# databricks/spark-sklearn

Measured on NVIDIA H100. Metric: candidate-fits/sec, higher is better.
Workload: dtype f64

## Files before the change

### include/b200gs.h

```cpp
#ifndef B200GS_H
#define B200GS_H

#include <stdint.h>

#ifdef __cplusplus
extern "C" {
#endif

typedef struct gs_handle gs_handle;

enum gs_status {
    GS_OK = 0,
    GS_ERR_CUDA = -1,
    GS_ERR_ARG = -2,
    GS_ERR_NO_DATA = -3,
    GS_ERR_UNSUPPORTED = -4,
    GS_ERR_NUMERIC = -5
};

enum gs_kernel { GS_KERNEL_LINEAR = 0, GS_KERNEL_RBF = 1 };
enum gs_dtype { GS_F32 = 0, GS_F64 = 1 };

enum gs_flags {
    GS_RETURN_TRAIN = 1,
// ... 52 lines not shown
                    double *coef_out, int32_t *n_iter);

int gs_set_targets_f64(gs_handle *h, const double *y);
int gs_svr(gs_handle *h, int32_t n_cand, const int32_t *kernel, const double *C, const double *epsilon, const double *gamma,
           double tol, int32_t max_iter, uint32_t flags, double *test_scores, double *train_scores, int32_t *n_iter,
           int32_t *n_sv, float *fit_ms, float *score_ms);
int gs_svr_refit(gs_handle *h, int32_t kernel, double C, double epsilon, double gamma, double tol, int32_t max_iter,
                 uint32_t flags, double *coef, double *rho, int32_t *n_iter);

int gs_debug_gram(gs_handle *h, double *S_out, double *xsq_out);
int gs_debug_kernel_matrix(gs_handle *h, int32_t kernel, double gamma, float *K_out);

int gs_debug_gemm_nt(gs_handle *h, const float *A, int32_t M, const float *B, int32_t N, int32_t K, float *C);

double gs_svc_predicted_iterations(int32_t kernel, double C, double gamma, int32_t d);
int32_t gs_svc_cluster_count(const double *cost_desc, int32_t n, int32_t sm_count);
void gs_svc_schedule(const double *cost_desc, int32_t n, int32_t sm_count, int32_t *n_cluster, int32_t *n_exclusive);
double gs_svc_simulate(const double *cost_desc, int32_t n, int32_t sm_count, int32_t n_cluster, int32_t n_exclusive);

typedef struct gs_profile {
    float ms_total;
    float ms_h2d;
    float ms_gram;
    float ms_kernel_matrix;
    float ms_solve;
    float ms_score;
    int64_t launches;
    int64_t smo_iterations;
    double solve_bytes;
    double gram_flops;
// ... 13 lines not shown
```

### spark_sklearn_b200/csrc/api.cu

```cuda
#include "common.cuh"
#include <algorithm>
#include <cmath>
#include <cstring>
#include <cstdio>
#include <cstdlib>
#include <map>
#include <mutex>
#include <queue>
#include <numeric>

static std::string g_create_error;

double gs_score_from_counts(int kind, int pos_class, int n_classes, const int *cnt)
{
    auto sup = [&](int c) { return (double)cnt[c * 3 + 0]; };
    auto tp = [&](int c) { return (double)cnt[c * 3 + 1]; };
    auto prd = [&](int c) { return (double)cnt[c * 3 + 2]; };
    auto f1c = [&](int c) { const double den = sup(c) + prd(c); return den > 0 ? 2.0 * tp(c) / den : 0.0; };
    double n = 0, correct = 0;
    for (int c = 0; c < n_classes; c++) { n += sup(c); correct += tp(c); }
    if (!(n > 0)) return NAN;
    switch (kind) {
    case GS_SCORE_DEFAULT: return correct / n;
    case GS_SCORE_BALANCED_ACCURACY: {
// ... 258 lines not shown
    GS_CUDA(cudaMemcpyAsync(h->dTe.p, h->te_mask.data(), (size_t)n * 16, cudaMemcpyHostToDevice, h->stream));
    GS_CUDA(cudaMemcpyAsync(h->dTr.p, h->tr_mask.data(), (size_t)n * 16, cudaMemcpyHostToDevice, h->stream));
    GS_CUDA(cudaStreamSynchronize(h->stream));
    h->prof.h2d_bytes += n * 32;
    return GS_OK;
}

extern "C" double gs_svc_predicted_iterations(int32_t kernel, double C, double gamma, int32_t d)
{
    if (kernel != GS_KERNEL_RBF) return C;
    const double gd = gamma * (double)d;
    if (!(gd > 0)) return C;
    return std::min(4.0 + 10.3 * std::pow(C * gd, 0.95), 9.0 + 7.3 / gd);
}

extern "C" int32_t gs_svc_cluster_count(const double *cost_desc, int32_t n, int32_t sm_count)
{
    if (!cost_desc || n < 2 || sm_count < 4) return 0;
    double total = 0;
    for (int q = 0; q < n; q++) total += cost_desc[q];
    const int nmax = std::min(n - 1, sm_count / 4);
    double best = 0, clustered = 0;
    int pick = 0;
    for (int k = 0; k <= nmax; k++) {
        const double f = std::max({(total + clustered) / sm_count, 0.9 * cost_desc[k], k > 0 ? 0.5 * cost_desc[0] : 0.0});
        if (k == 0 || f < 0.97 * best) { best = f; pick = k; }
        clustered += cost_desc[k];
    }
    return pick;
}
// ... 235 lines not shown
    if (!refit && h->score_kind != GS_SCORE_DEFAULT) {
        const int kd = h->score_kind;
        if (kd == GS_SCORE_NEG_MSE || kd == GS_SCORE_NEG_RMSE) { gs_set_error(h, "gs_svc: regression scorer on a classifier"); return GS_ERR_ARG; }
        if ((kd == GS_SCORE_ROC_AUC || kd == GS_SCORE_F1 || kd == GS_SCORE_PRECISION || kd == GS_SCORE_RECALL) && nc != 2) {
            gs_set_error(h, "gs_svc: this scorer is defined for binary problems only"); return GS_ERR_UNSUPPORTED;
        }
        if (h->score_pos >= nc) { gs_set_error(h, "gs_svc: positive class out of range"); return GS_ERR_ARG; }
    }
    int64_t total_iter = 0;
    double solve_bytes = 0;

    for (int g0 = 0; g0 < n_groups; g0 += gpb) {
        const int g1 = std::min(n_groups, g0 + gpb);
        if (const int rc = search.kernel_matrices(g0, g1)) return rc;
        std::vector<SmoProblem> probs;
        std::vector<int> prob_task, group_first(g1 - g0 + 1, 0);
        std::vector<VoteTask> vtasks;
        std::vector<int> vtask_id;
        for (int g = g0; g < g1; g++) {
            group_first[g - g0] = (int)probs.size();
            for (int t : search.group_tasks[g]) {
                const int c = t / n_splits, k = t % n_splits;
                vtasks.push_back(VoteTask{(int)probs.size(), refit ? -100 : k});
                vtask_id.push_back(t);
                for (int p = 0; p < n_pairs; p++) {
                    const size_t s = (size_t)k * n_pairs + p;
                    SmoProblem P;
                    memset(&P, 0, sizeof P);
                    P.K = h->dK.as<float>() + (size_t)(g - g0) * n * ldk;
                    P.qd = search.groups[g].first == GS_KERNEL_LINEAR ? h->dXsq.as<double>() : nullptr;
                    P.rows = d_rows + sp_off[s];
// ... 2 lines not shown
                    for (int e = 0; e < 4; e++) { P.seg_start[e] = sp_seg[s * 8 + e]; P.seg_len[e] = sp_seg[s * 8 + 4 + e]; }
                    P.n_pos = sp_npos[s];
                    P.ldk = ldk; P.C = Cv[c]; P.Cn = Cv[c]; P.eps = tol; P.max_iter = max_iter;
                    if (h->class_w_sets > 0) {
                        const double *cw = &h->class_w[(size_t)(h->class_w_sets == 1 ? 0 : k) * nc];
                        int a_ = 0, b_ = 0, q_ = 0;
                        for (int a = 0; a < nc; a++) for (int b = a + 1; b < nc; b++, q_++) if (q_ == p) { a_ = a; b_ = b; }
                        P.C = Cv[c] * cw[a_]; P.Cn = Cv[c] * cw[b_];
                    }
                    P.shrinking = (flags & GS_NO_SHRINKING) ? 0 : 1;
                    P.guard = search.d_guard;
                    P.nslots = 0;
                    for (int e = 0; e < P.nseg; e++) P.nslots += P.seg_len[e];
                    probs.push_back(P);
                    prob_task.push_back(t);
                }
            }
        }
        group_first[g1 - g0] = (int)probs.size();
        const int np = (int)probs.size();
        if (const int rc = search.workspaces(probs)) return rc;
        GS_CUDA(h->dWork[6].reserve((size_t)np * sizeof(SmoProblem) + (size_t)np * 4 + vtasks.size() * (sizeof(VoteTask) + 16) + 256));
        std::vector<double> cost(np);
        for (int q = 0; q < np; q++) {
            const int t = prob_task[q];
            const auto &grp = search.groups[search.task_group[t]];
            cost[q] = gs_svc_predicted_iterations(grp.first, Cv[t / n_splits], grp.second, (int32_t)d) * (double)probs[q].l;
        }
        std::vector<int> order(np);
        std::iota(order.begin(), order.end(), 0);
        std::stable_sort(order.begin(), order.end(), [&](int a, int b) { return cost[a] > cost[b]; });
        unsigned char *dmeta = h->dWork[6].as<unsigned char>();
        SmoProblem *d_probs = (SmoProblem *)dmeta;
        int *d_order = (int *)(dmeta + (size_t)np * sizeof(SmoProblem));
        size_t off = (size_t)np * sizeof(SmoProblem) + (size_t)np * 4;
        off = (off + 15) & ~(size_t)15;
        VoteTask *d_vt = (VoteTask *)(dmeta + off);
        off += vtasks.size() * sizeof(VoteTask);
        off = (off + 15) & ~(size_t)15;
        int *d_counts = (int *)(dmeta + off);
        GS_CUDA(cudaMemcpyAsync(d_probs, probs.data(), (size_t)np * sizeof(SmoProblem), cudaMemcpyHostToDevice, st));
        GS_CUDA(cudaMemcpyAsync(d_order, order.data(), (size_t)np * 4, cudaMemcpyHostToDevice, st));
        GS_CUDA(cudaMemcpyAsync(d_vt, vtasks.data(), vtasks.size() * sizeof(VoteTask), cudaMemcpyHostToDevice, st));
        GS_CUDA(cudaMemsetAsync(d_counts, 0, vtasks.size() * 16, st));
        GS_CUDA(cudaMemsetAsync(h->dWork[3].p, 0, (size_t)np * n * 8, st));
        pf.h2d_bytes += (size_t)np * sizeof(SmoProblem) + (size_t)np * 4 + vtasks.size() * sizeof(VoteTask);
        search.tm.mark(4);
        std::string why;
        int max_slots = 0;
        bool lean_ok = lmax < 16383 && !(getenv("B200GS_SMO_LEAN") && atoi(getenv("B200GS_SMO_LEAN")) == 0);
        for (int q = 0; q < np && lean_ok; q++) {
            lean_ok = probs[q].nseg > 0 && probs[q].nslots <= smo_lean_max_slots();
            max_slots = std::max(max_slots, probs[q].nslots);
        }
        auto launch_single = [&](const int *ord, int cnt, cudaStream_t s_, bool exclusive) -> cudaError_t {
            for (int inst = search.fast ? 1 : 0; inst >= 0; inst--) {
                const cudaError_t e = lean_ok ? launch_smo_lean(d_probs, ord, cnt, max_slots, inst == 1, exclusive, s_)
                                              : launch_smo(d_probs, ord, cnt, lmax, inst == 1, (int)ldk, s_, &why);
                if (e != cudaSuccess) return e;
                pf.launches++;
            }
            return cudaSuccess;
        };
        int cl = 0, n_cl = 0, n_ex = 0;
        if (lmax > 2048) {
            if (np * 8 <= h->sm_count) { cl = 8; n_cl = np; }
            else if (np * 4 <= h->sm_count) { cl = 4; n_cl = np; }
            else if (np * 2 <= h->sm_count) { cl = 2; n_cl = np; }
            else {
                std::vector<double> sorted_cost(np);
                for (int q = 0; q < np; q++) sorted_cost[q] = cost[order[q]];
                if (lean_ok) gs_svc_schedule(sorted_cost.data(), np, h->sm_count, &n_cl, &n_ex);
                else n_cl = gs_svc_cluster_count(sorted_cost.data(), np, h->sm_count);
                if (n_cl > 0) cl = 4;
            }
        }
        if (const char *e = getenv("B200GS_SMO_CLUSTER")) { cl = atoi(e); if (n_cl == 0) n_cl = std::max(1, np * 6 / 100); }
        if (const char *e = getenv("B200GS_SMO_CLUSTER_N")) n_cl = std::min(np, atoi(e));
        if (!(cl == 2 || cl == 4 || cl == 8) || lmax > smo_colown_max_rows(cl) || lmax <= 2048) n_cl = 0;
        if (const char *e = getenv("B200GS_SMO_EXCLUSIVE_N")) n_ex = atoi(e);
        if (!lean_ok) n_ex = 0;
        n_ex = std::max(0, std::min(n_ex, np - n_cl));
        if (n_cl > 0 || n_ex > 0) {
            cudaEvent_t ready = h->evp.get();
            cudaEventRecord(ready, st);
            cudaError_t ce = cudaSuccess;
            if (n_cl > 0) {
                for (int inst = search.fast ? 1 : 0; inst >= 0 && ce == cudaSuccess; inst--) {
                    ce = launch_smo_colown(d_probs, d_order, n_cl, lmax, cl, inst == 1, st);
                    pf.launches++;
                }
                if (ce != cudaSuccess) { gs_set_error(h, std::string("launch_smo_colown: ") + cudaGetErrorString(ce)); return GS_ERR_CUDA; }
            }
            if (n_ex > 0) {
                cudaEvent_t done = h->evp.get();
                cudaStreamWaitEvent(h->stream_hi, ready, 0);
                launch_delay(30000, h->stream_hi);
// ... 39 lines not shown
                GS_CUDA(cudaMemcpyAsync(score_raw.data(), d_auc, (size_t)nvt * 32, cudaMemcpyDeviceToHost, st));
            } else {
                GS_CUDA(h->dScore.reserve((size_t)nvt * 2 * nc * 3 * 4));
                GS_CUDA(cudaMemsetAsync(h->dScore.p, 0, (size_t)nvt * 2 * nc * 3 * 4, st));
                GS_CUDA(launch_vote_classes(h->dWork[4].as<double>(), search.d_rho, n, nc, h->dY.as<int>(), h->masks(),
                                            d_vt, nvt, h->dScore.as<int>(), st));
                class_counts.resize((size_t)nvt * 2 * nc * 3);
                GS_CUDA(cudaMemcpyAsync(class_counts.data(), h->dScore.p, class_counts.size() * 4, cudaMemcpyDeviceToHost, st));
            }
            pf.launches++;
        }
        search.tm.mark(3);
        std::vector<int> counts(vtasks.size() * 4);
        GS_CUDA(cudaMemcpyAsync(counts.data(), d_counts, counts.size() * 4, cudaMemcpyDeviceToHost, st));
        pf.d2h_bytes += counts.size() * 4;
        if (const int rc = search.results(np, refit && pair_coef)) return rc;
        const auto &info = search.info; const auto &ns = search.ns; const auto &rho = search.rho;
        for (int q = 0; q < np; q++) {
            const int t = prob_task[q];
            task_iter[t] += info[(size_t)q * 4]; task_sv[t] += info[(size_t)q * 4 + 2];
            task_fit_ms[t] += (double)(ns[(size_t)q * 12 + 1] - ns[(size_t)q * 12]) * 1e-6;
            total_iter += info[(size_t)q * 4];
            solve_bytes += (double)info[(size_t)q * 4] * 2.0 * probs[q].l * 4.0;
            if (!std::isfinite(rho[q])) { if (refit) { gs_set_error(h, "gs_svc_refit: non-finite intercept"); return GS_ERR_NUMERIC; } task_bad[t] = 1; }
        }
        if (getenv("B200GS_SMO_TIMELINE") && atoi(getenv("B200GS_SMO_TIMELINE"))) {
            unsigned long long t0 = ~0ull;
            for (int q = 0; q < np; q++) if (ns[(size_t)q * 12]) t0 = std::min(t0, ns[(size_t)q * 12]);
            auto span = [&](int a, int b, const char *name) {
                if (b <= a) return;
                double s0 = 1e30, s1 = 0, e0 = 1e30, e1 = 0; long long it_max = 0;
                for (int i = a; i < b; i++) {
                    const int q = order[i];
                    const double st_ = (double)(ns[(size_t)q * 12] - t0) * 1e-6, en = (double)(ns[(size_t)q * 12 + 1] - t0) * 1e-6;
                    s0 = std::min(s0, st_); s1 = std::max(s1, st_); e0 = std::min(e0, en); e1 = std::max(e1, en);
                    it_max = std::max<long long>(it_max, info[(size_t)q * 4]);
                }
                fprintf(stderr, "[timeline] %-9s %4d problems: starts %.2f..%.2f ms, ends %.2f..%.2f ms, longest %lld iterations\n",
                        name, b - a, s0, s1, e0, e1, it_max);
            };
            span(0, n_cl, "cluster"); span(n_cl, n_cl + n_ex, "exclusive"); span(n_cl + n_ex, np, "shared");
            for (int i = 0; i < std::min(np, 16); i++) {
                const int q = order[i];
                fprintf(stderr, "[timeline]   #%d: %d iterations, %.2f -> %.2f ms (%.3f us/iteration)\n", i, info[(size_t)q * 4],
                        (double)(ns[(size_t)q * 12] - t0) * 1e-6, (double)(ns[(size_t)q * 12 + 1] - t0) * 1e-6,
                        (double)(ns[(size_t)q * 12 + 1] - ns[(size_t)q * 12]) * 1e-3 / std::max(1, info[(size_t)q * 4]));
            }
        }
        if (getenv("B200GS_SMO_PROF") && atoi(getenv("B200GS_SMO_PROF"))) {
            int qmax = 0;
            for (int q = 1; q < np; q++) if (info[(size_t)q * 4] > info[(size_t)qmax * 4]) qmax = q;
            const unsigned long long *pn = &ns[(size_t)qmax * 12];
            const double it = (double)info[(size_t)qmax * 4];
            fprintf(stderr, "[smo prof] longest problem: %d iters, %.1f ms (%.2f us/iter); cycles/iter by slot:", info[(size_t)qmax * 4],
                    (double)(pn[1] - pn[0]) * 1e-6, (double)(pn[1] - pn[0]) * 1e-3 / it);
            for (int e = 0; e < 10; e++) fprintf(stderr, " %.0f", pn[2 + e] / it);
// ... 116 lines not shown
```

### spark_sklearn_b200/csrc/common.cuh

```cuda
#pragma once
#include <cuda_runtime.h>
#include <stdint.h>
#include <cstring>
#include <string>
#include <vector>
#include "../../include/b200gs.h"

#define GS_CUDA(call)                                                                         \
    do {                                                                                      \
        cudaError_t e_ = (call);                                                              \
        if (e_ != cudaSuccess) {                                                              \
            gs_set_error(h, std::string(#call) + ": " + cudaGetErrorString(e_) + " @" +       \
                                __FILE__ + ":" + std::to_string(__LINE__));                   \
            return GS_ERR_CUDA;                                                               \
        }                                                                                     \
    } while (0)

struct DevBuf {
    void *p = nullptr;
    size_t cap = 0;
    cudaError_t reserve(size_t bytes)
    {
        if (bytes <= cap) return cudaSuccess;
        if (p) cudaFree(p);
// ... 109 lines not shown
    DevBuf dSw;
    std::vector<double> z64;
    DevBuf dZ64;
    gs_profile prof;
    EventPool evp;
    TensorTimer tt;
};

void gs_set_error(gs_handle *h, const std::string &msg);

cudaError_t launch_gram_f64(const void *X, int x_dtype, int n, int d, double *S, double *xsq, cudaStream_t st);
cudaError_t launch_widen_gram(const float *S32, int n, int64_t ld32, double *S, double *xsq, cudaStream_t st);
cudaError_t launch_kernel_matrix(const double *S, const double *xsq, int n, int kernel, double gamma,
                                 float *K, int64_t ldk, int *special, cudaStream_t st);

struct SmoProblem {
    const float *K;
    const double *qd;
    const int *rows;
    double *alpha;
    double *Gbar;
    int *scratch;
    double *coef;
    double *out_rho;
    int *out_info;
    unsigned long long *out_ns;
    const int *guard;
    int64_t ldk;
    double C, Cn, eps;
    int l, n_pos, max_iter, shrinking;
    int nseg, seg_start[4], seg_len[4];
    int nslots;
};
cudaError_t launch_smo(const SmoProblem *d_probs, const int *d_order, int n_prob, int lmax, bool fast, int rowcap,
                       cudaStream_t st, std::string *why);
int smo_max_rows();
struct SvrData {
    const double *z;
    double eps;
};
cudaError_t launch_smo_svr(const SmoProblem *d_probs, const SvrData *d_svr, const int *d_order, int n_prob, int lmax, bool fast,
                           int rowcap, cudaStream_t st, std::string *why);
int smo_lean_max_slots();
cudaError_t launch_smo_lean(const SmoProblem *d_probs, const int *d_order, int n_prob, int max_slots, bool fast, bool exclusive, cudaStream_t st);
int smo_colown_max_rows(int cl);
void launch_delay(unsigned ns, cudaStream_t st);
cudaError_t launch_smo_colown(const SmoProblem *d_probs, const int *d_order, int n_prob, int lmax, int cl, bool fast, cudaStream_t st);

int decision_chunks(int n, int ncols, int sms);
cudaError_t launch_decision(const double *S, const double *xsq, int n, int kernel, double gamma,
                            const double *coef, int ncols, double *dec, double *part, int jchunks, cudaStream_t st);
struct VoteTask {
    int first_col;
    int fold;
};
cudaError_t launch_vote(const double *dec, const double *rho, int n, int n_classes, const int *y,
                        SplitMasks sm, const VoteTask *tasks, int n_tasks, int *counts,
                        cudaStream_t st);

// ... 58 lines not shown
```

### spark_sklearn_b200/csrc/smo_common.cuh

```cuda
#pragma once
#include "common.cuh"
#include <math_constants.h>

namespace smo {

constexpr double TAU = 1e-12;
constexpr int ST_LOWER = 0, ST_UPPER = 1, ST_FREE = 2;
constexpr int F_YPOS = 4, F_UP = 8, F_LOW = 16, F_MARK = 32;
constexpr int IDX_SHIFT = 5;
constexpr int SAFETY_MAX_ITER = 10000000;

__device__ __forceinline__ int mkflags(bool ypos, int st)
{
    const bool up = ypos ? st != ST_UPPER : st != ST_LOWER;
    const bool low = ypos ? st != ST_LOWER : st != ST_UPPER;
    return st | (ypos ? F_YPOS : 0) | (up ? F_UP : 0) | (low ? F_LOW : 0);
}

__device__ __forceinline__ unsigned long long dkey(double x)
{
    const long long u = __double_as_longlong(x);
    return (unsigned long long)u ^ ((unsigned long long)(u >> 63) | 0x8000000000000000ull);
}
__device__ __forceinline__ double dkey_inv(unsigned long long k)
// ... 68 lines not shown
    __syncthreads();
    if (lane == 0) cnt[w] = __popc(b);
    __syncthreads();
    int base = 0, tot = 0;
#pragma unroll
    for (int i = 0; i < NT / 32; i++) {
        const int c = cnt[i];
        if (i < w) base += c;
        tot += c;
    }
    total = tot;
    return base + __popc(b & ((1u << lane) - 1u));
}


}
```

### spark_sklearn_b200/csrc/smo_lean.cu

```cuda
#include "smo_common.cuh"
#include <algorithm>
#include <cstdlib>
#include <type_traits>

namespace {

using namespace smo;

constexpr unsigned LF_UP = 4u, LF_LOW = 8u;
constexpr int POS_SHIFT = 18, SLOT_SHIFT = 4;
constexpr unsigned SLOT_MASK = 0x3fffu;
constexpr unsigned PF_INERT = 0xfffffff0u;

__device__ __forceinline__ unsigned lean_flags(bool ypos, int st)
{
    const bool up = ypos ? st != ST_UPPER : st != ST_LOWER;
    const bool low = ypos ? st != ST_LOWER : st != ST_UPPER;
    return (unsigned)st | (up ? LF_UP : 0u) | (low ? LF_LOW : 0u);
}

template <int N, int I = 0, class F>
__device__ __forceinline__ void lean_loop(F &&f)
{
    if constexpr (I < N) { f(std::integral_constant<int, I>{}); lean_loop<N, I + 1>(f); }
// ... 69 lines not shown
                 : "+d"(m), "+d"(la), "+r"(la_k), "+r"(tie)
                 : "r"(__float_as_uint(kvi)), "r"(__float_as_uint(kvj)), "d"(a), "d"(b), "r"(fm), "n"(1u << (2 * K)), "n"(K));
}

struct LeanRed {
    unsigned a_hi[32], a_lo[32], a_pf[32];
    unsigned b_k1[32], b_pf[32], b_k2[32], b_fl[32];
    float b_kq[32]; double b_al[32], b_mg[32];
    double al_i;
    double bc_d[4]; int bc_i[2];
    unsigned x_hi[32], x_lo[32], x_pf[32];
    float x_kq[32]; double x_al[32], x_mg[32];
    double dm[32], dm2[32]; int cnt[32];
    int seg_slot[5], seg_col[4];
    int ysplit;
};

template <int NT, int G, bool FAST, bool PROF, bool SOLO>
__global__ void __launch_bounds__(NT, (NT * G >= 4096 || NT >= 1024 ? 1 : 2048 / (NT * G / 2) > 8 ? 8 : 2048 / (NT * G / 2)))
smo_lean_kernel(const SmoProblem *__restrict__ probs, const int *__restrict__ order)
{
    extern __shared__ __align__(16) unsigned char smem_raw[];
    __shared__ LeanRed red;
    constexpr int NW = NT / 32;
    constexpr int KPT = G * 4;
    constexpr int LCAP = NT * KPT;

    const SmoProblem *__restrict__ Pp = probs + order[blockIdx.x];
    if (Pp->guard != nullptr && (*Pp->guard != 0) == FAST) return;
    const int tid = threadIdx.x, lane = tid & 31, warp = tid >> 5;
    const int l = Pp->l;
    const int nslots = Pp->nslots;
    double *const mG = reinterpret_cast<double *>(smem_raw);
    unsigned *const pfS = reinterpret_cast<unsigned *>(mG + LCAP);
    double *const alpha_g = Pp->alpha;
    double *const gbar_g = Pp->Gbar;
    int *const scratch = Pp->scratch;
    const float *__restrict__ const K = Pp->K;
    const int64_t ldk = Pp->ldk;
    const double eps = Pp->eps;
    const double Cc = Pp->C, Cneg = Pp->Cn;
    const bool use_gbar = Pp->shrinking != 0;
    const double *__restrict__ const qd = FAST ? nullptr : Pp->qd;

    unsigned long long t_start = 0;
    if (tid == 0) asm volatile("mov.u64 %0, %%globaltimer;" : "=l"(t_start));

    if (tid == 0) {
        int s = 0;
        for (int e = 0; e < 4; e++) {
            red.seg_slot[e] = e < Pp->nseg ? s : 0x7fffffff;
            red.seg_col[e] = e < Pp->nseg ? Pp->seg_start[e] : 0;
            if (e < Pp->nseg) s += Pp->seg_len[e];
        }
        red.seg_slot[4] = 0x7fffffff;
    }
    __syncthreads();
    auto slot_col = [&](int slot) -> int {
        const int e = (slot >= red.seg_slot[1]) + (slot >= red.seg_slot[2]) + (slot >= red.seg_slot[3]);
        return red.seg_col[e] + (slot - red.seg_slot[e]);
    };
    int gcol[G];
#pragma unroll
// ... 450 lines not shown
                *reinterpret_cast<uint4 *>(pfS + s4) = make_uint4(pv[0], pv[1], pv[2], pv[3]);
            }
            active = na;
        }
        refresh_flags();
        __syncthreads();
    };

    refresh_flags();
    bool scan_valid = false, second = false;
    for (;;) {
        if (!second) {
            if (iter >= max_iter) { timed_out = 1; break; }
            if (--counter == 0) {
                counter = l < 1000 ? l : 1000;
                if (use_gbar) { do_shrink(); scan_valid = false; }
                if constexpr (PROF) tprev = clock64();
            }
        }
        if (!scan_valid) local_scan();
        if (select()) {
            if (second) break;
            rebuild_gradient();
            active = l;
            refresh_flags();
            __syncthreads();
            scan_valid = false;
            second = true;
            continue;
        }
        if (second) { counter = 1; second = false; }
        ++iter;

        const int slot_i = (int)((pi >> SLOT_SHIFT) & SLOT_MASK), slot_j = (int)((pj >> SLOT_SHIFT) & SLOT_MASK);
        float kvj[KPT];
        load_row(col_j, kvj);
        double a = 0, b = 0, ai_new = 0, aj_new = 0;
        int sti = 0, stj = 0;
        const bool yi = slot_i < ysplit, yj = slot_j < ysplit;
        if (SOLO || warp == 0) {
            const double Ci = yi ? Cc : Cneg, Cj = yj ? Cc : Cneg;
            const double Gi = yi ? -gmax : gmax;
            const double Gj = yj ? -mg_j : mg_j;
            const double QDi = QDc(col_i), QDj = QDc(col_j);
            const double Qij = (yi == yj) ? k_ij : -k_ij;
            double ai = alpha_i, aj = alpha_j;
            if (yi != yj) {
                double quad = __dadd_rn(__dadd_rn(QDi, QDj), __dmul_rn(2.0, Qij));
                if (quad <= 0) quad = TAU;
                const double delta = __ddiv_rn(__dsub_rn(-Gi, Gj), quad);
                const double diff = __dsub_rn(ai, aj);
                ai = __dadd_rn(ai, delta); aj = __dadd_rn(aj, delta);
                if (diff > 0) { if (aj < 0) { aj = 0; ai = diff; } }
                else          { if (ai < 0) { ai = 0; aj = -diff; } }
                if (diff > __dsub_rn(Ci, Cj)) { if (ai > Ci) { ai = Ci; aj = __dsub_rn(Ci, diff); } }
                else                          { if (aj > Cj) { aj = Cj; ai = __dadd_rn(Cj, diff); } }
            } else {
                double quad = __dsub_rn(__dadd_rn(QDi, QDj), __dmul_rn(2.0, Qij));
                if (quad <= 0) quad = TAU;
                const double delta = __ddiv_rn(__dsub_rn(Gi, Gj), quad);
                const double sum = __dadd_rn(ai, aj);
                ai = __dsub_rn(ai, delta); aj = __dadd_rn(aj, delta);
                if (sum > Ci) { if (ai > Ci) { ai = Ci; aj = __dsub_rn(sum, Ci); } }
                else         { if (aj < 0) { aj = 0; ai = sum; } }
                if (sum > Cj) { if (aj > Cj) { aj = Cj; ai = __dsub_rn(sum, Cj); } }
                else         { if (ai < 0) { ai = 0; aj = sum; } }
            }
            const double dai = __dsub_rn(ai, alpha_i), daj = __dsub_rn(aj, alpha_j);
            sti = ai >= Ci ? ST_UPPER : (ai <= 0 ? ST_LOWER : ST_FREE);
            stj = aj >= Cj ? ST_UPPER : (aj <= 0 ? ST_LOWER : ST_FREE);
            a = yi ? -dai : dai;
            b = yj ? -daj : daj;
            ai_new = ai; aj_new = aj;
            if constexpr (!SOLO) {
                if (lane == 0) {
                    red.bc_d[0] = a; red.bc_d[1] = b; red.bc_d[2] = ai; red.bc_d[3] = aj;
                    red.bc_i[0] = sti; red.bc_i[1] = stj;
                }
            }
        }
        tick(4);
        if constexpr (!SOLO) {
// ... 95 lines not shown
            const int s4 = (g * NT + tid) * 4;
            double mv[4]; unsigned pv[4];
            load_m4(s4, mv); load_pf4(s4, pv);
#pragma unroll
            for (int q = 0; q < 4; q++) {
                yg[g * 4 + q] = -mv[q]; wv[g * 4 + q] = pv[q];
                if (pv[q] < PF_INERT) {
                    const double av = __ldcg(alpha_g + s4 + q);
                    coef[gcol[g] + q] = s4 + q < ysplit ? av : -av;
                    nsv += av > 0;
                    nbsv += av >= (s4 + q < ysplit ? Cc : Cneg);
                }
            }
        }
    }
    __syncthreads();
    {
        const unsigned act_lim = (unsigned)active << POS_SHIFT;
#pragma unroll
        for (int k = 0; k < KPT; k++) {
            if (wv[k] < act_lim) {
                const int p = (int)(wv[k] >> POS_SHIFT);
                const int s = ((k >> 2) * NT + tid) * 4 + (k & 3);
                mG[p] = yg[k];
                pfS[p] = (wv[k] & 3u) | (s < ysplit ? 4u : 0u);
            }
        }
    }
    __syncthreads();
    if (tid == 0) {
// ... 14 lines not shown
        nbsv += __shfl_xor_sync(0xffffffffu, nbsv, s);
    }
    if (lane == 0) { red.cnt[warp] = nsv; red.a_pf[warp] = (unsigned)nbsv; }
    __syncthreads();
    if (tid == 0) {
        int s = 0, bs = 0;
        for (int w = 0; w < NW; w++) { s += red.cnt[w]; bs += (int)red.a_pf[w]; }
        int *info = Pp->out_info;
        info[0] = iter; info[1] = timed_out; info[2] = s; info[3] = bs;
        unsigned long long t_end;
        asm volatile("mov.u64 %0, %%globaltimer;" : "=l"(t_end));
        unsigned long long *ns = Pp->out_ns;
        ns[0] = t_start; ns[1] = t_end;
        if constexpr (PROF)
            for (int q = 0; q < 8; q++) ns[2 + q] = (unsigned long long)prof[q];
    }
}

template <int NT, int G, bool FAST, bool PROF, bool SOLO>
cudaError_t launch_lean_one(const SmoProblem *probs, const int *order, int n_prob, bool exclusive, cudaStream_t st)
{
    constexpr int LCAP = NT * G * 4;
    const size_t smem = exclusive ? std::max<size_t>((size_t)LCAP * 12, 132 * 1024) : (size_t)LCAP * 12;
    auto kern = smo_lean_kernel<NT, G, FAST, PROF, SOLO>;
    cudaError_t e = cudaFuncSetAttribute(kern, cudaFuncAttributeMaxDynamicSharedMemorySize, (int)smem);
    if (e != cudaSuccess) return e;
    e = cudaFuncSetAttribute(kern, cudaFuncAttributePreferredSharedMemoryCarveout, cudaSharedmemCarveoutMaxShared);
    if (e != cudaSuccess) return e;
    kern<<<n_prob, NT, smem, st>>>(probs, order);
    return cudaGetLastError();
}

template <int NT, int G, bool SOLO>
cudaError_t launch_lean_cfg2(const SmoProblem *probs, const int *order, int n_prob, bool fast, bool prof, bool excl, cudaStream_t st)
{
    if (prof) return fast ? launch_lean_one<NT, G, true, true, SOLO>(probs, order, n_prob, excl, st) : launch_lean_one<NT, G, false, true, SOLO>(probs, order, n_prob, excl, st);
    return fast ? launch_lean_one<NT, G, true, false, SOLO>(probs, order, n_prob, excl, st) : launch_lean_one<NT, G, false, false, SOLO>(probs, order, n_prob, excl, st);
}

template <int NT, int G>
cudaError_t launch_lean_cfg(const SmoProblem *probs, const int *order, int n_prob, bool fast, bool prof, bool excl, bool solo, cudaStream_t st)
{
    return solo ? launch_lean_cfg2<NT, G, true>(probs, order, n_prob, fast, prof, excl, st) : launch_lean_cfg2<NT, G, false>(probs, order, n_prob, fast, prof, excl, st);
}

int env_int(const char *name, int dflt)
{
    const char *v = getenv(name);
    return v && *v ? atoi(v) : dflt;
}

}

int smo_lean_max_slots() { return 16384; }

cudaError_t launch_smo_lean(const SmoProblem *d_probs, const int *d_order, int n_prob, int max_slots, bool fast, bool exclusive, cudaStream_t st)
{
    if (n_prob <= 0) return cudaSuccess;
    const bool prof = env_int("B200GS_SMO_PROF", 0) != 0;
    if (env_int("B200GS_SMO_NOFAST", 0)) fast = false;
    bool solo = false;
    if (const char *e = getenv("B200GS_LEAN_SOLO")) solo = atoi(e) != 0;
    if (exclusive && max_slots > 4096 && max_slots <= 8192 && env_int("B200GS_LEAN_EXCL_WIDE", 1))
        return launch_lean_cfg<1024, 2>(d_probs, d_order, n_prob, fast, prof, exclusive, solo, st);
    if (max_slots <= 2048) return launch_lean_cfg<128, 4>(d_probs, d_order, n_prob, fast, prof, exclusive, solo, st);
    if (max_slots <= 4096) return launch_lean_cfg<256, 4>(d_probs, d_order, n_prob, fast, prof, exclusive, solo, st);
    if (max_slots <= 8192) return launch_lean_cfg<512, 4>(d_probs, d_order, n_prob, fast, prof, exclusive, solo, st);
    if (max_slots <= 16384) return launch_lean_cfg<1024, 4>(d_probs, d_order, n_prob, fast, prof, exclusive, solo, st);
    return cudaErrorInvalidValue;
}
```

### spark_sklearn_b200/engine.py

```python
import ctypes
import os

import numpy as np

_HERE = os.path.dirname(os.path.abspath(__file__))
LIB_PATH = os.path.join(_HERE, "libb200gs.so")

GS_RETURN_TRAIN, GS_GRAM_TENSOR, GS_NO_SHRINKING = 1, 2, 4
KERNEL_ID = {"linear": 0, "rbf": 1}

_lib = None


class GsProfile(ctypes.Structure):
    _fields_ = [("ms_total", ctypes.c_float), ("ms_h2d", ctypes.c_float), ("ms_gram", ctypes.c_float),
                ("ms_kernel_matrix", ctypes.c_float), ("ms_solve", ctypes.c_float), ("ms_score", ctypes.c_float),
                ("launches", ctypes.c_int64), ("smo_iterations", ctypes.c_int64),
                ("solve_bytes", ctypes.c_double), ("gram_flops", ctypes.c_double), ("gram_bytes", ctypes.c_double),
                ("h2d_bytes", ctypes.c_int64), ("d2h_bytes", ctypes.c_int64),
                ("ms_tensor", ctypes.c_float), ("tensor_flops", ctypes.c_double)]


class EngineError(RuntimeError):
    def __init__(self, status, msg):
# ... 33 lines not shown
    L.gs_ridge.argtypes = [vp, i32, vp, i32, u32, vp, vp, vp, vp]
    L.gs_ridge_refit.argtypes = [vp, dbl, i32, vp]
    L.gs_enet.argtypes = [vp, i32, vp, vp, i32, dbl, i32, u32, vp, vp, vp, vp, vp]
    L.gs_enet_refit.argtypes = [vp, dbl, dbl, i32, dbl, i32, vp, vp, vp]
    L.gs_set_targets_f64.argtypes = [vp, vp]
    L.gs_svr.argtypes = [vp, i32, vp, vp, vp, vp, dbl, i32, u32, vp, vp, vp, vp, vp, vp]
    L.gs_svr_refit.argtypes = [vp, i32, dbl, dbl, dbl, dbl, i32, u32, vp, vp, vp]
    L.gs_logreg.argtypes = [vp, i32, vp, dbl, i32, i32, u32, vp, vp, vp, vp, vp]
    L.gs_logreg_refit.argtypes = [vp, dbl, dbl, i32, i32, vp, vp]
    L.gs_get_profile.argtypes = [vp, c.POINTER(GsProfile)]
    L.gs_debug_gram.argtypes = [vp, vp, vp]
    L.gs_debug_kernel_matrix.argtypes = [vp, i32, dbl, vp]
    L.gs_debug_gemm_nt.argtypes = [vp, vp, i32, vp, i32, i32, vp]
    L.gs_svc_predicted_iterations.argtypes = [i32, dbl, dbl, i32]
    L.gs_svc_predicted_iterations.restype = dbl
    L.gs_svc_cluster_count.argtypes = [vp, i32, i32]
    L.gs_svc_cluster_count.restype = i32
    L.gs_svc_schedule.argtypes = [vp, i32, i32, vp, vp]
    L.gs_svc_schedule.restype = None
    L.gs_svc_simulate.argtypes = [vp, i32, i32, i32, i32]
    L.gs_svc_simulate.restype = dbl
    for f in ("gs_create", "gs_set_data", "gs_svc", "gs_svc_refit", "gs_ridge", "gs_ridge_refit", "gs_enet", "gs_enet_refit", "gs_set_targets_f64",
              "gs_svr", "gs_svr_refit", "gs_logreg",
              "gs_logreg_refit", "gs_get_profile", "gs_debug_gram", "gs_debug_kernel_matrix", "gs_debug_gemm_nt"):
        getattr(L, f).restype = c.c_int
    _lib = L
    return L


def _ptr(a):
# ... 210 lines not shown
```

Before: 862.4.

## Chain SVC solves across C values and copy leader solution when bound never binds

Within a grid search, SVC problems that share a kernel, fold and class pair but differ only in C are linked to the largest-C leader. The leader publishes a certificate, the largest alpha value its SMO steps ever tested, with a release store. A follower with smaller C polls it with an acquire load and, if its own C exceeds that value, copies the leader's coefficients instead of solving. The scheduler now orders followers after non-followers and stops chaining any follower whose leader runs on a cluster. This cuts redundant SMO iterations at the cost of extra kernel template variants, periodic polling and cross-block memory ordering risk.

```diff
diff --git a/include/b200gs.h b/include/b200gs.h
--- a/include/b200gs.h
+++ b/include/b200gs.h
@@ -90,6 +90,7 @@
 int gs_debug_gemm_nt(gs_handle *h, const float *A, int32_t M, const float *B, int32_t N, int32_t K, float *C);
 
 double gs_svc_predicted_iterations(int32_t kernel, double C, double gamma, int32_t d);
+int32_t gs_svc_predicted_copy(int32_t kernel, double C, double C_lead, double gamma, int32_t d);
 int32_t gs_svc_cluster_count(const double *cost_desc, int32_t n, int32_t sm_count);
 void gs_svc_schedule(const double *cost_desc, int32_t n, int32_t sm_count, int32_t *n_cluster, int32_t *n_exclusive);
 double gs_svc_simulate(const double *cost_desc, int32_t n, int32_t sm_count, int32_t n_cluster, int32_t n_exclusive);
diff --git a/spark_sklearn_b200/csrc/api.cu b/spark_sklearn_b200/csrc/api.cu
--- a/spark_sklearn_b200/csrc/api.cu
+++ b/spark_sklearn_b200/csrc/api.cu
@@ -1,5 +1,7 @@
 #include "common.cuh"
 #include <algorithm>
+#include <array>
+#include <functional>
 #include <cmath>
 #include <cstring>
 #include <cstdio>
@@ -296,6 +298,14 @@
     return std::min(4.0 + 10.3 * std::pow(C * gd, 0.95), 9.0 + 7.3 / gd);
 }
 
+extern "C" int32_t gs_svc_predicted_copy(int32_t kernel, double C, double C_lead, double gamma, int32_t d)
+{
+    const double gd = gamma * (double)d;
+    if (kernel != GS_KERNEL_RBF || !(gd > 0) || !(C < C_lead)) return 0;
+    const double onset = std::pow((5.0 + 7.3 / gd) / 10.3, 1.0 / 0.95) / gd;
+    return C >= 7.0 * onset ? 1 : 0;
+}
+
 extern "C" int32_t gs_svc_cluster_count(const double *cost_desc, int32_t n, int32_t sm_count)
 {
     if (!cost_desc || n < 2 || sm_count < 4) return 0;
@@ -561,7 +571,7 @@
         const int g1 = std::min(n_groups, g0 + gpb);
         if (const int rc = search.kernel_matrices(g0, g1)) return rc;
         std::vector<SmoProblem> probs;
-        std::vector<int> prob_task, group_first(g1 - g0 + 1, 0);
+        std::vector<int> prob_task, prob_pair, group_first(g1 - g0 + 1, 0);
         std::vector<VoteTask> vtasks;
         std::vector<int> vtask_id;
         for (int g = g0; g < g1; g++) {
@@ -594,22 +604,74 @@
                     for (int e = 0; e < P.nseg; e++) P.nslots += P.seg_len[e];
                     probs.push_back(P);
                     prob_task.push_back(t);
+                    prob_pair.push_back(p);
                 }
             }
         }
         group_first[g1 - g0] = (int)probs.size();
         const int np = (int)probs.size();
         if (const int rc = search.workspaces(probs)) return rc;
-        GS_CUDA(h->dWork[6].reserve((size_t)np * sizeof(SmoProblem) + (size_t)np * 4 + vtasks.size() * (sizeof(VoteTask) + 16) + 256));
+        GS_CUDA(h->dWork[6].reserve((size_t)np * (sizeof(SmoProblem) + 4 + sizeof(SmoCert)) + vtasks.size() * (sizeof(VoteTask) + 16) + 256));
+        int max_slots = 0;
+        bool lean_ok = lmax < 16383 && !(getenv("B200GS_SMO_LEAN") && atoi(getenv("B200GS_SMO_LEAN")) == 0);
+        for (int q = 0; q < np && lean_ok; q++) {
+            lean_ok = probs[q].nseg > 0 && probs[q].nslots <= smo_lean_max_slots();
+            max_slots = std::max(max_slots, probs[q].nslots);
+        }
         std::vector<double> cost(np);
         for (int q = 0; q < np; q++) {
             const int t = prob_task[q];
             const auto &grp = search.groups[search.task_group[t]];
             cost[q] = gs_svc_predicted_iterations(grp.first, Cv[t / n_splits], grp.second, (int32_t)d) * (double)probs[q].l;
         }
+        const bool chains = lean_ok && !(lmax > 2048 && np * 2 <= h->sm_count);
+        std::vector<int> lead(np, -1);
+        if (chains) {
+            std::map<std::array<int, 3>, int> top;
+            auto key = [&](int q) { const int t = prob_task[q]; return std::array<int, 3>{search.task_group[t], t % n_splits, prob_pair[q]}; };
+            for (int q = 0; q < np; q++) {
+                if (probs[q].C != probs[q].Cn) continue;
+                auto it = top.emplace(key(q), q).first;
+                if (probs[q].C > probs[it->second].C) it->second = q;
+            }
+            for (int q = 0; q < np; q++) {
+                if (probs[q].C != probs[q].Cn) continue;
+                const int L = top[key(q)];
+                const auto &grp = search.groups[search.task_group[prob_task[q]]];
+                if (gs_svc_predicted_copy(grp.first, probs[q].C, probs[L].C, grp.second, (int32_t)d)) lead[q] = L;
+            }
+        }
+        std::string why;
+        int cl = 0, n_cl = 0, n_ex = 0;
+        if (lmax > 2048) {
+            if (np * 8 <= h->sm_count) { cl = 8; n_cl = np; }
+            else if (np * 4 <= h->sm_count) { cl = 4; n_cl = np; }
+            else if (np * 2 <= h->sm_count) { cl = 2; n_cl = np; }
+            else {
+                std::vector<double> sorted_cost(cost);
+                for (int q = 0; q < np; q++) if (lead[q] >= 0) sorted_cost[q] = 0.0;
+                std::sort(sorted_cost.begin(), sorted_cost.end(), std::greater<double>());
+                if (lean_ok) gs_svc_schedule(sorted_cost.data(), np, h->sm_count, &n_cl, &n_ex);
+                else n_cl = gs_svc_cluster_count(sorted_cost.data(), np, h->sm_count);
+                if (n_cl > 0) cl = 4;
+            }
+        }
+        if (const char *e = getenv("B200GS_SMO_CLUSTER")) { cl = atoi(e); if (n_cl == 0) n_cl = std::max(1, np * 6 / 100); }
+        if (const char *e = getenv("B200GS_SMO_CLUSTER_N")) n_cl = std::min(np, atoi(e));
+        if (!(cl == 2 || cl == 4 || cl == 8) || lmax > smo_colown_max_rows(cl) || lmax <= 2048) n_cl = 0;
+        if (const char *e = getenv("B200GS_SMO_EXCLUSIVE_N")) n_ex = atoi(e);
+        if (!lean_ok) n_ex = 0;
+        n_ex = std::max(0, std::min(n_ex, np - n_cl));
         std::vector<int> order(np);
         std::iota(order.begin(), order.end(), 0);
-        std::stable_sort(order.begin(), order.end(), [&](int a, int b) { return cost[a] > cost[b]; });
+        for (bool again = true; again;) {
+            std::stable_sort(order.begin(), order.end(), [&](int a, int b) { return (lead[a] < 0) != (lead[b] < 0) ? lead[a] < 0 : cost[a] > cost[b]; });
+            std::vector<char> on_cluster(np, 0);
+            for (int i = 0; i < n_cl; i++) on_cluster[order[i]] = 1;
+            again = false;
+            for (int q = 0; q < np; q++)
+                if (lead[q] >= 0 && on_cluster[lead[q]]) { lead[q] = -1; again = true; }
+        }
         unsigned char *dmeta = h->dWork[6].as<unsigned char>();
         SmoProblem *d_probs = (SmoProblem *)dmeta;
         int *d_order = (int *)(dmeta + (size_t)np * sizeof(SmoProblem));
@@ -619,6 +681,15 @@
         off += vtasks.size() * sizeof(VoteTask);
         off = (off + 15) & ~(size_t)15;
         int *d_counts = (int *)(dmeta + off);
+        off += vtasks.size() * 16;
+        SmoCert *d_cert = (SmoCert *)(dmeta + off);
+        if (chains) {
+            for (int q = 0; q < np; q++) {
+                probs[q].cert = d_cert + q;
+                probs[q].lead = lead[q] >= 0 ? d_probs + lead[q] : nullptr;
+            }
+            GS_CUDA(cudaMemsetAsync(d_cert, 0xff, (size_t)np * sizeof(SmoCert), st));
+        }
         GS_CUDA(cudaMemcpyAsync(d_probs, probs.data(), (size_t)np * sizeof(SmoProblem), cudaMemcpyHostToDevice, st));
         GS_CUDA(cudaMemcpyAsync(d_order, order.data(), (size_t)np * 4, cudaMemcpyHostToDevice, st));
         GS_CUDA(cudaMemcpyAsync(d_vt, vtasks.data(), vtasks.size() * sizeof(VoteTask), cudaMemcpyHostToDevice, st));
@@ -626,41 +697,15 @@
         GS_CUDA(cudaMemsetAsync(h->dWork[3].p, 0, (size_t)np * n * 8, st));
         pf.h2d_bytes += (size_t)np * sizeof(SmoProblem) + (size_t)np * 4 + vtasks.size() * sizeof(VoteTask);
         search.tm.mark(4);
-        std::string why;
-        int max_slots = 0;
-        bool lean_ok = lmax < 16383 && !(getenv("B200GS_SMO_LEAN") && atoi(getenv("B200GS_SMO_LEAN")) == 0);
-        for (int q = 0; q < np && lean_ok; q++) {
-            lean_ok = probs[q].nseg > 0 && probs[q].nslots <= smo_lean_max_slots();
-            max_slots = std::max(max_slots, probs[q].nslots);
-        }
         auto launch_single = [&](const int *ord, int cnt, cudaStream_t s_, bool exclusive) -> cudaError_t {
             for (int inst = search.fast ? 1 : 0; inst >= 0; inst--) {
-                const cudaError_t e = lean_ok ? launch_smo_lean(d_probs, ord, cnt, max_slots, inst == 1, exclusive, s_)
+                const cudaError_t e = lean_ok ? launch_smo_lean(d_probs, ord, cnt, max_slots, inst == 1, exclusive, chains, s_)
                                               : launch_smo(d_probs, ord, cnt, lmax, inst == 1, (int)ldk, s_, &why);
                 if (e != cudaSuccess) return e;
                 pf.launches++;
             }
             return cudaSuccess;
         };
-        int cl = 0, n_cl = 0, n_ex = 0;
-        if (lmax > 2048) {
-            if (np * 8 <= h->sm_count) { cl = 8; n_cl = np; }
-            else if (np * 4 <= h->sm_count) { cl = 4; n_cl = np; }
-            else if (np * 2 <= h->sm_count) { cl = 2; n_cl = np; }
-            else {
-                std::vector<double> sorted_cost(np);
-                for (int q = 0; q < np; q++) sorted_cost[q] = cost[order[q]];
-                if (lean_ok) gs_svc_schedule(sorted_cost.data(), np, h->sm_count, &n_cl, &n_ex);
-                else n_cl = gs_svc_cluster_count(sorted_cost.data(), np, h->sm_count);
-                if (n_cl > 0) cl = 4;
-            }
-        }
-        if (const char *e = getenv("B200GS_SMO_CLUSTER")) { cl = atoi(e); if (n_cl == 0) n_cl = std::max(1, np * 6 / 100); }
-        if (const char *e = getenv("B200GS_SMO_CLUSTER_N")) n_cl = std::min(np, atoi(e));
-        if (!(cl == 2 || cl == 4 || cl == 8) || lmax > smo_colown_max_rows(cl) || lmax <= 2048) n_cl = 0;
-        if (const char *e = getenv("B200GS_SMO_EXCLUSIVE_N")) n_ex = atoi(e);
-        if (!lean_ok) n_ex = 0;
-        n_ex = std::max(0, std::min(n_ex, np - n_cl));
         if (n_cl > 0 || n_ex > 0) {
             cudaEvent_t ready = h->evp.get();
             cudaEventRecord(ready, st);
@@ -730,14 +775,23 @@
         std::vector<int> counts(vtasks.size() * 4);
         GS_CUDA(cudaMemcpyAsync(counts.data(), d_counts, counts.size() * 4, cudaMemcpyDeviceToHost, st));
         pf.d2h_bytes += counts.size() * 4;
+        std::vector<SmoCert> cert(chains ? np : 0);
+        if (chains) {
+            GS_CUDA(cudaMemcpyAsync(cert.data(), d_cert, (size_t)np * sizeof(SmoCert), cudaMemcpyDeviceToHost, st));
+            pf.d2h_bytes += (size_t)np * sizeof(SmoCert);
+        }
         if (const int rc = search.results(np, refit && pair_coef)) return rc;
         const auto &info = search.info; const auto &ns = search.ns; const auto &rho = search.rho;
+        int n_follow = 0, n_copied = 0;
         for (int q = 0; q < np; q++) {
             const int t = prob_task[q];
             task_iter[t] += info[(size_t)q * 4]; task_sv[t] += info[(size_t)q * 4 + 2];
             task_fit_ms[t] += (double)(ns[(size_t)q * 12 + 1] - ns[(size_t)q * 12]) * 1e-6;
-            total_iter += info[(size_t)q * 4];
-            solve_bytes += (double)info[(size_t)q * 4] * 2.0 * probs[q].l * 4.0;
+            const int executed = chains ? cert[q].executed : info[(size_t)q * 4];
+            n_follow += lead[q] >= 0;
+            n_copied += chains && cert[q].copied == 1;
+            total_iter += executed;
+            solve_bytes += (double)executed * 2.0 * probs[q].l * 4.0;
             if (!std::isfinite(rho[q])) { if (refit) { gs_set_error(h, "gs_svc_refit: non-finite intercept"); return GS_ERR_NUMERIC; } task_bad[t] = 1; }
         }
         if (getenv("B200GS_SMO_TIMELINE") && atoi(getenv("B200GS_SMO_TIMELINE"))) {
@@ -756,6 +810,7 @@
                         name, b - a, s0, s1, e0, e1, it_max);
             };
             span(0, n_cl, "cluster"); span(n_cl, n_cl + n_ex, "exclusive"); span(n_cl + n_ex, np, "shared");
+            fprintf(stderr, "[timeline] solve chains: %d followers, %d copied, %d solved\n", n_follow, n_copied, n_follow - n_copied);
             for (int i = 0; i < std::min(np, 16); i++) {
                 const int q = order[i];
                 fprintf(stderr, "[timeline]   #%d: %d iterations, %.2f -> %.2f ms (%.3f us/iteration)\n", i, info[(size_t)q * 4],
diff --git a/spark_sklearn_b200/csrc/common.cuh b/spark_sklearn_b200/csrc/common.cuh
--- a/spark_sklearn_b200/csrc/common.cuh
+++ b/spark_sklearn_b200/csrc/common.cuh
@@ -147,6 +147,11 @@
 cudaError_t launch_kernel_matrix(const double *S, const double *xsq, int n, int kernel, double gamma,
                                  float *K, int64_t ldk, int *special, cudaStream_t st);
 
+struct SmoCert {
+    unsigned long long m;
+    int executed;
+    int copied;
+};
 struct SmoProblem {
     const float *K;
     const double *qd;
@@ -164,6 +169,8 @@
     int l, n_pos, max_iter, shrinking;
     int nseg, seg_start[4], seg_len[4];
     int nslots;
+    SmoCert *cert;
+    const SmoProblem *lead;
 };
 cudaError_t launch_smo(const SmoProblem *d_probs, const int *d_order, int n_prob, int lmax, bool fast, int rowcap,
                        cudaStream_t st, std::string *why);
@@ -175,7 +182,8 @@
 cudaError_t launch_smo_svr(const SmoProblem *d_probs, const SvrData *d_svr, const int *d_order, int n_prob, int lmax, bool fast,
                            int rowcap, cudaStream_t st, std::string *why);
 int smo_lean_max_slots();
-cudaError_t launch_smo_lean(const SmoProblem *d_probs, const int *d_order, int n_prob, int max_slots, bool fast, bool exclusive, cudaStream_t st);
+cudaError_t launch_smo_lean(const SmoProblem *d_probs, const int *d_order, int n_prob, int max_slots, bool fast, bool exclusive, bool chain,
+                            cudaStream_t st);
 int smo_colown_max_rows(int cl);
 void launch_delay(unsigned ns, cudaStream_t st);
 cudaError_t launch_smo_colown(const SmoProblem *d_probs, const int *d_order, int n_prob, int lmax, int cl, bool fast, cudaStream_t st);
diff --git a/spark_sklearn_b200/csrc/smo_common.cuh b/spark_sklearn_b200/csrc/smo_common.cuh
--- a/spark_sklearn_b200/csrc/smo_common.cuh
+++ b/spark_sklearn_b200/csrc/smo_common.cuh
@@ -106,4 +106,34 @@
 }
 
 
+__device__ __forceinline__ void cert_publish(const SmoProblem *P, double M, int executed)
+{
+    P->cert->executed = executed;
+    P->cert->copied = 0;
+    asm volatile("st.release.gpu.global.u64 [%0], %1;" ::"l"(&P->cert->m), "l"((unsigned long long)__double_as_longlong(M)) : "memory");
 }
+
+__device__ __forceinline__ bool cert_covers(const SmoProblem *P)
+{
+    unsigned long long v;
+    asm volatile("ld.acquire.gpu.global.u64 %0, [%1];" : "=l"(v) : "l"(&P->lead->cert->m) : "memory");
+    return __longlong_as_double((long long)v) < P->C;
+}
+
+static __device__ __noinline__ void cert_copy(const SmoProblem *P, int executed, unsigned long long t_start)
+{
+    const SmoProblem *L = P->lead;
+    const int *__restrict__ rows = P->rows;
+    for (int p = threadIdx.x; p < P->l; p += blockDim.x) P->coef[rows[p]] = __ldcg(L->coef + rows[p]);
+    if (threadIdx.x == 0) {
+        *P->out_rho = __ldcg(L->out_rho);
+        for (int k = 0; k < 4; k++) P->out_info[k] = __ldcg(L->out_info + k);
+        P->cert->executed = executed;
+        P->cert->copied = 1;
+        unsigned long long t_end;
+        asm volatile("mov.u64 %0, %%globaltimer;" : "=l"(t_end));
+        P->out_ns[0] = t_start; P->out_ns[1] = t_end;
+    }
+}
+
+}
diff --git a/spark_sklearn_b200/csrc/smo_lean.cu b/spark_sklearn_b200/csrc/smo_lean.cu
--- a/spark_sklearn_b200/csrc/smo_lean.cu
+++ b/spark_sklearn_b200/csrc/smo_lean.cu
@@ -107,9 +107,11 @@
     double dm[32], dm2[32]; int cnt[32];
     int seg_slot[5], seg_col[4];
     int ysplit;
+    int follow, copy;
+    double cert_m;
 };
 
-template <int NT, int G, bool FAST, bool PROF, bool SOLO>
+template <int NT, int G, bool FAST, bool PROF, bool SOLO, bool CHAIN>
 __global__ void __launch_bounds__(NT, (NT * G >= 4096 || NT >= 1024 ? 1 : 2048 / (NT * G / 2) > 8 ? 8 : 2048 / (NT * G / 2)))
 smo_lean_kernel(const SmoProblem *__restrict__ probs, const int *__restrict__ order)
 {
@@ -138,8 +140,19 @@
 
     unsigned long long t_start = 0;
     if (tid == 0) asm volatile("mov.u64 %0, %%globaltimer;" : "=l"(t_start));
+    auto lead_covers = [&]() -> bool {
+        if (tid == 0) red.copy = cert_covers(Pp);
+        __syncthreads();
+        return red.copy != 0;
+    };
+    if constexpr (CHAIN) {
+        if (tid == 0) red.follow = Pp->lead != nullptr;
+        __syncthreads();
+        if (red.follow && lead_covers()) { cert_copy(Pp, 0, t_start); return; }
+    }
 
     if (tid == 0) {
+        if constexpr (CHAIN) red.cert_m = 0.0;
         int s = 0;
         for (int e = 0; e < 4; e++) {
             red.seg_slot[e] = e < Pp->nseg ? s : 0x7fffffff;
@@ -620,6 +633,7 @@
             if (iter >= max_iter) { timed_out = 1; break; }
             if (--counter == 0) {
                 counter = l < 1000 ? l : 1000;
+                if constexpr (CHAIN) if (red.follow && lead_covers()) { cert_copy(Pp, iter, t_start); return; }
                 if (use_gbar) { do_shrink(); scan_valid = false; }
                 if constexpr (PROF) tprev = clock64();
             }
@@ -650,7 +664,7 @@
             const double Gj = yj ? -mg_j : mg_j;
             const double QDi = QDc(col_i), QDj = QDc(col_j);
             const double Qij = (yi == yj) ? k_ij : -k_ij;
-            double ai = alpha_i, aj = alpha_j;
+            double ai = alpha_i, aj = alpha_j, tested;
             if (yi != yj) {
                 double quad = __dadd_rn(__dadd_rn(QDi, QDj), __dmul_rn(2.0, Qij));
                 if (quad <= 0) quad = TAU;
@@ -659,6 +673,7 @@
                 ai = __dadd_rn(ai, delta); aj = __dadd_rn(aj, delta);
                 if (diff > 0) { if (aj < 0) { aj = 0; ai = diff; } }
                 else          { if (ai < 0) { ai = 0; aj = -diff; } }
+                tested = fmax(ai, aj);
                 if (diff > __dsub_rn(Ci, Cj)) { if (ai > Ci) { ai = Ci; aj = __dsub_rn(Ci, diff); } }
                 else                          { if (aj > Cj) { aj = Cj; ai = __dadd_rn(Cj, diff); } }
             } else {
@@ -671,7 +686,9 @@
                 else         { if (aj < 0) { aj = 0; ai = sum; } }
                 if (sum > Cj) { if (aj > Cj) { aj = Cj; ai = __dsub_rn(sum, Cj); } }
                 else         { if (ai < 0) { ai = 0; aj = sum; } }
-            }
+                tested = fmax(sum, fmax(ai, aj));
+            }
+            if constexpr (CHAIN) if (tid == 0) red.cert_m = fmax(red.cert_m, tested);
             const double dai = __dsub_rn(ai, alpha_i), daj = __dsub_rn(aj, alpha_j);
             sti = ai >= Ci ? ST_UPPER : (ai <= 0 ? ST_LOWER : ST_FREE);
             stj = aj >= Cj ? ST_UPPER : (aj <= 0 ? ST_LOWER : ST_FREE);
@@ -797,6 +814,7 @@
             }
         }
     }
+    if constexpr (CHAIN) __threadfence();
     __syncthreads();
     {
         const unsigned act_lim = (unsigned)active << POS_SHIFT;
@@ -841,15 +859,16 @@
         ns[0] = t_start; ns[1] = t_end;
         if constexpr (PROF)
             for (int q = 0; q < 8; q++) ns[2 + q] = (unsigned long long)prof[q];
-    }
-}
-
-template <int NT, int G, bool FAST, bool PROF, bool SOLO>
+        if constexpr (CHAIN) { __threadfence(); cert_publish(Pp, red.cert_m, iter); }
+    }
+}
+
+template <int NT, int G, bool FAST, bool PROF, bool SOLO, bool CHAIN>
 cudaError_t launch_lean_one(const SmoProblem *probs, const int *order, int n_prob, bool exclusive, cudaStream_t st)
 {
     constexpr int LCAP = NT * G * 4;
     const size_t smem = exclusive ? std::max<size_t>((size_t)LCAP * 12, 132 * 1024) : (size_t)LCAP * 12;
-    auto kern = smo_lean_kernel<NT, G, FAST, PROF, SOLO>;
+    auto kern = smo_lean_kernel<NT, G, FAST, PROF, SOLO, CHAIN>;
     cudaError_t e = cudaFuncSetAttribute(kern, cudaFuncAttributeMaxDynamicSharedMemorySize, (int)smem);
     if (e != cudaSuccess) return e;
     e = cudaFuncSetAttribute(kern, cudaFuncAttributePreferredSharedMemoryCarveout, cudaSharedmemCarveoutMaxShared);
@@ -858,17 +877,23 @@
     return cudaGetLastError();
 }
 
+template <int NT, int G, bool SOLO, bool CHAIN>
+cudaError_t launch_lean_cfg3(const SmoProblem *probs, const int *order, int n_prob, bool fast, bool prof, bool excl, cudaStream_t st)
+{
+    if (prof) return fast ? launch_lean_one<NT, G, true, true, SOLO, CHAIN>(probs, order, n_prob, excl, st) : launch_lean_one<NT, G, false, true, SOLO, CHAIN>(probs, order, n_prob, excl, st);
+    return fast ? launch_lean_one<NT, G, true, false, SOLO, CHAIN>(probs, order, n_prob, excl, st) : launch_lean_one<NT, G, false, false, SOLO, CHAIN>(probs, order, n_prob, excl, st);
+}
+
 template <int NT, int G, bool SOLO>
-cudaError_t launch_lean_cfg2(const SmoProblem *probs, const int *order, int n_prob, bool fast, bool prof, bool excl, cudaStream_t st)
-{
-    if (prof) return fast ? launch_lean_one<NT, G, true, true, SOLO>(probs, order, n_prob, excl, st) : launch_lean_one<NT, G, false, true, SOLO>(probs, order, n_prob, excl, st);
-    return fast ? launch_lean_one<NT, G, true, false, SOLO>(probs, order, n_prob, excl, st) : launch_lean_one<NT, G, false, false, SOLO>(probs, order, n_prob, excl, st);
+cudaError_t launch_lean_cfg2(const SmoProblem *probs, const int *order, int n_prob, bool fast, bool prof, bool excl, bool chain, cudaStream_t st)
+{
+    return chain ? launch_lean_cfg3<NT, G, SOLO, true>(probs, order, n_prob, fast, prof, excl, st) : launch_lean_cfg3<NT, G, SOLO, false>(probs, order, n_prob, fast, prof, excl, st);
 }
 
 template <int NT, int G>
-cudaError_t launch_lean_cfg(const SmoProblem *probs, const int *order, int n_prob, bool fast, bool prof, bool excl, bool solo, cudaStream_t st)
-{
-    return solo ? launch_lean_cfg2<NT, G, true>(probs, order, n_prob, fast, prof, excl, st) : launch_lean_cfg2<NT, G, false>(probs, order, n_prob, fast, prof, excl, st);
+cudaError_t launch_lean_cfg(const SmoProblem *probs, const int *order, int n_prob, bool fast, bool prof, bool excl, bool solo, bool chain, cudaStream_t st)
+{
+    return solo ? launch_lean_cfg2<NT, G, true>(probs, order, n_prob, fast, prof, excl, chain, st) : launch_lean_cfg2<NT, G, false>(probs, order, n_prob, fast, prof, excl, chain, st);
 }
 
 int env_int(const char *name, int dflt)
@@ -881,7 +906,8 @@
 
 int smo_lean_max_slots() { return 16384; }
 
-cudaError_t launch_smo_lean(const SmoProblem *d_probs, const int *d_order, int n_prob, int max_slots, bool fast, bool exclusive, cudaStream_t st)
+cudaError_t launch_smo_lean(const SmoProblem *d_probs, const int *d_order, int n_prob, int max_slots, bool fast, bool exclusive, bool chain,
+                            cudaStream_t st)
 {
     if (n_prob <= 0) return cudaSuccess;
     const bool prof = env_int("B200GS_SMO_PROF", 0) != 0;
@@ -889,10 +915,10 @@
     bool solo = false;
     if (const char *e = getenv("B200GS_LEAN_SOLO")) solo = atoi(e) != 0;
     if (exclusive && max_slots > 4096 && max_slots <= 8192 && env_int("B200GS_LEAN_EXCL_WIDE", 1))
-        return launch_lean_cfg<1024, 2>(d_probs, d_order, n_prob, fast, prof, exclusive, solo, st);
-    if (max_slots <= 2048) return launch_lean_cfg<128, 4>(d_probs, d_order, n_prob, fast, prof, exclusive, solo, st);
-    if (max_slots <= 4096) return launch_lean_cfg<256, 4>(d_probs, d_order, n_prob, fast, prof, exclusive, solo, st);
-    if (max_slots <= 8192) return launch_lean_cfg<512, 4>(d_probs, d_order, n_prob, fast, prof, exclusive, solo, st);
-    if (max_slots <= 16384) return launch_lean_cfg<1024, 4>(d_probs, d_order, n_prob, fast, prof, exclusive, solo, st);
+        return launch_lean_cfg<1024, 2>(d_probs, d_order, n_prob, fast, prof, exclusive, solo, chain, st);
+    if (max_slots <= 2048) return launch_lean_cfg<128, 4>(d_probs, d_order, n_prob, fast, prof, exclusive, solo, chain, st);
+    if (max_slots <= 4096) return launch_lean_cfg<256, 4>(d_probs, d_order, n_prob, fast, prof, exclusive, solo, chain, st);
+    if (max_slots <= 8192) return launch_lean_cfg<512, 4>(d_probs, d_order, n_prob, fast, prof, exclusive, solo, chain, st);
+    if (max_slots <= 16384) return launch_lean_cfg<1024, 4>(d_probs, d_order, n_prob, fast, prof, exclusive, solo, chain, st);
     return cudaErrorInvalidValue;
 }
diff --git a/spark_sklearn_b200/engine.py b/spark_sklearn_b200/engine.py
--- a/spark_sklearn_b200/engine.py
+++ b/spark_sklearn_b200/engine.py
@@ -71,6 +71,8 @@
     L.gs_debug_gemm_nt.argtypes = [vp, vp, i32, vp, i32, i32, vp]
     L.gs_svc_predicted_iterations.argtypes = [i32, dbl, dbl, i32]
     L.gs_svc_predicted_iterations.restype = dbl
+    L.gs_svc_predicted_copy.argtypes = [i32, dbl, dbl, dbl, i32]
+    L.gs_svc_predicted_copy.restype = i32
     L.gs_svc_cluster_count.argtypes = [vp, i32, i32]
     L.gs_svc_cluster_count.restype = i32
     L.gs_svc_schedule.argtypes = [vp, i32, i32, vp, vp]
```

After: 919.1 (median of 6 runs). +6.6%, better.
